# kmaninis/OSVOS-PyTorch

Hardware: NVIDIA H100
Metric: frames/sec at 480x854 fwd-only, batch 1 per GPU (OSVOS.forward -> 5 logit maps) (higher is better)
Workload: dtype bf16x3 (split-bf16 operands, fp32 accumulate)

## Files before the change

osvos_pytorch_b200/csrc/common.cuh:

```cuda
#pragma once
#include <cuda.h>
#include <cuda_bf16.h>
#include <cuda_runtime.h>
#include <stdint.h>
#include <stdio.h>
#include <string.h>

#include "../../include/osvos_b200.h"

namespace osvos {

#define OSVOS_CHECK_ARG(cond)                                                              \
  do {                                                                                     \
    if (!(cond)) {                                                                         \
      set_last_error("%s:%d: invalid argument: %s", __FILE__, __LINE__, #cond);            \
      return OSVOS_ERR_INVALID_ARGUMENT;                                                   \
    }                                                                                      \
  } while (0)

#define OSVOS_CHECK_CUDA(expr)                                                             \
  do {                                                                                     \
    cudaError_t e__ = (expr);                                                              \
    if (e__ != cudaSuccess) {                                                              \
      set_last_error("%s:%d: %s -> %s", __FILE__, __LINE__, #expr, cudaGetErrorString(e__)); \
      return OSVOS_ERR_CUDA;                                                               \
    }                                                                                      \
  } while (0)

void set_last_error(const char* fmt, ...);

int encode_tensor_map(CUtensorMap* map, CUtensorMapDataType dtype, int elem_bytes, int rank, const void* base,
                      const uint64_t* dims, const uint64_t* strides_bytes, const uint32_t* box,
                      CUtensorMapSwizzle swizzle);

int device_sm_count();

bool pdl_enabled();

template <typename... KArgs, typename... Args>
static inline cudaError_t launch_pdl(void (*kern)(KArgs...), dim3 grid, dim3 block, size_t smem, cudaStream_t stream,
                                     Args&&... args) {
  cudaLaunchConfig_t cfg;
  memset(&cfg, 0, sizeof(cfg));
  cfg.gridDim = grid;
  cfg.blockDim = block;
  cfg.dynamicSmemBytes = smem;
  cfg.stream = stream;
  cudaLaunchAttribute attr[1];
  attr[0].id = cudaLaunchAttributeProgrammaticStreamSerialization;
  attr[0].val.programmaticStreamSerializationAllowed = 1;
  cfg.attrs = attr;
  cfg.numAttrs = pdl_enabled() ? 1 : 0;
  return cudaLaunchKernelEx(&cfg, kern, static_cast<KArgs>(args)...);
}

template <typename K>
static inline cudaError_t ensure_dynamic_smem(K kern, int bytes, uint64_t* done_mask) {
  int dev = 0;
  cudaError_t e = cudaGetDevice(&dev);
  if (e != cudaSuccess) return e;
  if (dev < 64 && ((*done_mask >> dev) & 1ull)) return cudaSuccess;
  e = cudaFuncSetAttribute(kern, cudaFuncAttributeMaxDynamicSharedMemorySize, bytes);
  if (e == cudaSuccess && dev < 64) *done_mask |= 1ull << dev;
  return e;
}

__device__ __forceinline__ void split_bf16(float v, __nv_bfloat16& hi, __nv_bfloat16& lo) {
  hi = __float2bfloat16_rn(v);
  lo = __float2bfloat16_rn(v - __bfloat162float(hi));
}
__device__ __forceinline__ uint32_t pack_bf16x2(__nv_bfloat16 a, __nv_bfloat16 b) {
  return static_cast<uint32_t>(__bfloat16_as_ushort(a)) | (static_cast<uint32_t>(__bfloat16_as_ushort(b)) << 16);
}
__device__ __forceinline__ bool last_block_arrives(unsigned int* counter) {
  __shared__ bool is_last;
  __threadfence();
  __syncthreads();
  if (threadIdx.x == 0) is_last = atomicAdd(counter, 1u) == gridDim.x * gridDim.y - 1;
  __syncthreads();
  if (is_last) __threadfence();
  return is_last;
}

template <typename T>
__device__ __forceinline__ T block_ordered_sum(const T* rows, int nrows, size_t stride, T* red ) {
  T t = T(0);
  for (int r = threadIdx.x; r < nrows; r += blockDim.x) t += __ldcg(rows + static_cast<size_t>(r) * stride);
  __syncthreads();
  red[threadIdx.x] = t;
  __syncthreads();
  T s = T(0);
  if (threadIdx.x == 0)
    for (int i = 0; i < static_cast<int>(blockDim.x); ++i) s += red[i];
  return s;
}

__device__ __forceinline__ float bf16_lo_to_float(uint32_t packed) { return __uint_as_float(packed << 16); }
__device__ __forceinline__ float bf16_hi_to_float(uint32_t packed) { return __uint_as_float(packed & 0xFFFF0000u); }

}
```

osvos_pytorch_b200/csrc/conv3x3_halo.cu:

```cuda
#include "conv_common.cuh"

namespace osvos {

constexpr int kHaloRows = kTileH + 2;
constexpr int kPitch = kTileW + 2;

template <int BLOCK_N, int PLANES, bool SPLIT>
struct HaloCfg {
  static constexpr int kABoxBytes = kHaloRows * kPitch * 128;
  static constexpr int kAPlaneBytes = (kABoxBytes + 1023) / 1024 * 1024;
  static constexpr int kAStageBytes = PLANES * kAPlaneBytes;
  static constexpr int kAStages = 2;
  static constexpr int kBPlaneBytes = BLOCK_N * 128;
  static constexpr int kBStageBytes = PLANES * kBPlaneBytes;
  static constexpr int kBudget = 225 * 1024 - kAStages * kAStageBytes;
  static constexpr int kBStagesRaw = kBudget / kBStageBytes;
  static constexpr int kBStages = kBStagesRaw > 9 ? 9 : kBStagesRaw;
  static constexpr bool kSplitAcc = SPLIT;
  static_assert(!SPLIT || (PLANES == 2 && BLOCK_N <= 128), "split accumulators need two planes and 2 * BLOCK_N <= 256");
  static constexpr int kAccCols = kSplitAcc ? 2 * BLOCK_N : BLOCK_N;
  static constexpr int kAcc = kAccCols / 2;
  static constexpr int kSmemBytes = kAStages * kAStageBytes + kBStages * kBStageBytes + 1024 + 512;
  static_assert(kBStages >= 2, "weight ring too shallow");
  static_assert(kSmemBytes <= 227 * 1024, "more than the per-CTA shared memory of sm_90");
  static_assert(kSmemBytes + 4096 < (1 << 18), "descriptor start-address field would overflow");
  static_assert(kBStageBytes % 1024 == 0, "B stage must keep 1024-byte alignment");
};

template <int BLOCK_N, int PLANES, bool SPLIT, bool LEAN, bool PINGPONG, bool DET = false>
__global__ void __launch_bounds__(kConvThreads, 1)
conv3x3_halo_kernel(const __grid_constant__ CUtensorMap map_x_hi, const __grid_constant__ CUtensorMap map_x_lo,
                    const __grid_constant__ CUtensorMap map_w_hi, const __grid_constant__ CUtensorMap map_w_lo,
                    const ConvParams p) {
  using Cfg = HaloCfg<BLOCK_N, PLANES, SPLIT>;
  constexpr int SA = Cfg::kAStages, SB = Cfg::kBStages;
  constexpr int kHalves = PINGPONG ? 2 : 1;
  static_assert(!PINGPONG || kHalves * Cfg::kAcc <= 128, "a ping-pong warpgroup holds the whole tile's accumulator");

  extern __shared__ uint8_t smem_raw[];
  uint8_t* smem = reinterpret_cast<uint8_t*>((reinterpret_cast<uintptr_t>(smem_raw) + 1023) & ~uintptr_t(1023));
  uint8_t* smem_a = smem;
  uint8_t* smem_b = smem + SA * Cfg::kAStageBytes;
  uint64_t* bars = reinterpret_cast<uint64_t*>(smem_b + SB * Cfg::kBStageBytes);
  uint64_t* a_full = bars;
  uint64_t* a_empty = bars + SA;
  uint64_t* b_full = bars + 2 * SA;
  uint64_t* b_empty = bars + 2 * SA + SB;

  const int warp = threadIdx.x >> 5;
  const int lane = threadIdx.x & 31;

  if (warp == 0 && lane == 0) {
    tma_prefetch_desc(&map_x_hi);
    tma_prefetch_desc(&map_w_hi);
    if (PLANES == 2) {
      tma_prefetch_desc(&map_x_lo);
      tma_prefetch_desc(&map_w_lo);
    }
    constexpr uint32_t kReaders = PINGPONG ? 1 : 2;
    for (int i = 0; i < SA; ++i) {
      mbar_init(&a_full[i], 1);
      mbar_init(&a_empty[i], kReaders);
    }
    for (int i = 0; i < SB; ++i) {
      mbar_init(&b_full[i], 1);
      mbar_init(&b_empty[i], kReaders);
    }
    fence_barrier_init();
  }
  __syncthreads();
  pdl_wait();
  pdl_launch_dependents();

  if (warp < 4) {
    if (PINGPONG) setmaxnreg_dec<40>();
    if (warp != 0) return;
    if (elect_one()) {
      int a_stage = 0, b_stage = 0;
      uint32_t a_phase = 0, b_phase = 0;
      const bool skip_a = (p.ablate & 2) != 0, skip_b = (p.ablate & 1) != 0;
      auto issue_a = [&](int x0, int y0, int img, int kc) {
        mbar_wait(&a_empty[a_stage], a_phase ^ 1);
        if (skip_a) {
          mbar_arrive(&a_full[a_stage]);
        } else {
          uint8_t* st = smem_a + a_stage * Cfg::kAStageBytes;
          mbar_arrive_expect_tx(&a_full[a_stage], PLANES * Cfg::kABoxBytes);
          tma_load_4d(&map_x_hi, &a_full[a_stage], st, kc * kBlockK, x0, y0, img);
          if (PLANES == 2) tma_load_4d(&map_x_lo, &a_full[a_stage], st + Cfg::kAPlaneBytes, kc * kBlockK, x0, y0, img);
        }
        if (++a_stage == SA) {
          a_stage = 0;
          a_phase ^= 1;
        }
      };
      int nb = 0, tx = 0, ty = 0, img = 0;
      const int w_first = static_cast<int>(blockIdx.x), w_stride = static_cast<int>(gridDim.x);
      if (w_first < p.total_tiles) {
        decode_tile(p, w_first, nb, tx, ty, img);
        issue_a(tx * kTileW - 1, ty * kTileH - 1, img, 0);
      }
      for (int tile = w_first; tile < p.total_tiles; tile += w_stride) {
        const bool has_next = tile + w_stride < p.total_tiles;
        int nnb = 0, ntx = 0, nty = 0, nimg = 0;
        if (has_next) decode_tile(p, tile + w_stride, nnb, ntx, nty, nimg);
        const int n0 = nb * BLOCK_N;
        for (int kc = 0; kc < p.k_chunks; ++kc) {
          const int c0 = kc * kBlockK;
#pragma unroll
          for (int tap = 0; tap < 9; ++tap) {
            if (tap == 3) {
              if (kc + 1 < p.k_chunks) issue_a(tx * kTileW - 1, ty * kTileH - 1, img, kc + 1);
              else if (has_next) issue_a(ntx * kTileW - 1, nty * kTileH - 1, nimg, 0);
            }
            mbar_wait(&b_empty[b_stage], b_phase ^ 1);
            if (skip_b) {
              mbar_arrive(&b_full[b_stage]);
            } else {
              uint8_t* st = smem_b + b_stage * Cfg::kBStageBytes;
              mbar_arrive_expect_tx(&b_full[b_stage], Cfg::kBStageBytes);
              tma_load_3d(&map_w_hi, &b_full[b_stage], st, c0, n0, tap);
              if (PLANES == 2) tma_load_3d(&map_w_lo, &b_full[b_stage], st + Cfg::kBPlaneBytes, c0, n0, tap);
            }
            if (++b_stage == SB) {
              b_stage = 0;
              b_phase ^= 1;
            }
          }
        }
        nb = nnb, tx = ntx, ty = nty, img = nimg;
      }
    }
    __syncwarp();
  } else {
    if (PINGPONG) setmaxnreg_inc<232>();
    const int wg = (warp - 4) >> 2, wl = warp & 3;
    const bool leader = (threadIdx.x & 127) == 0;
    constexpr uint64_t kDescA = desc_template(16, kPitch * 128, kDescSW128);
    constexpr uint64_t kDescB = desc_template(16, 1024, kDescSW128);
    constexpr uint32_t kLoPlaneA = Cfg::kAPlaneBytes >> 4, kLoPlaneB = Cfg::kBPlaneBytes >> 4;
    constexpr uint32_t kHalfA = (8 * kPitch * 128) >> 4;
    const uint32_t smem_a_u32 = smem_u32(smem_a) + (PINGPONG ? 0 : wg * 8 * kPitch * 128), smem_b_u32 = smem_u32(smem_b);
    const bool skip_mma = (p.ablate & 4) != 0;
    float acc[kHalves][Cfg::kAcc];
    StageRelease pending;
    constexpr int kOwners = PINGPONG ? 2 : 1;
    for (int k = PINGPONG ? wg : 0;; k += kOwners) {
      const int tile = static_cast<int>(blockIdx.x) + k * static_cast<int>(gridDim.x);
      if (tile >= p.total_tiles) break;
      const bool has_next = tile + static_cast<int>(gridDim.x) < p.total_tiles;
      const int a_seq = k * p.k_chunks, b_seq = 9 * a_seq;
      int a_stage = a_seq % SA, b_stage = b_seq % SB;
      uint32_t a_phase = (a_seq / SA) & 1, b_phase = (b_seq / SB) & 1;
      if (PINGPONG && k > 0) named_bar_sync(1 + wg, 256);
#pragma unroll
      for (int h = 0; h < kHalves; ++h)
#pragma unroll
        for (int i = 0; i < Cfg::kAcc; ++i) acc[h][i] = 0.f;
      for (int kc = 0; kc < p.k_chunks; ++kc) {
        mbar_wait(&a_full[a_stage], a_phase);
        const uint64_t da0 = kDescA | static_cast<uint64_t>((smem_a_u32 + a_stage * Cfg::kAStageBytes) >> 4);
#pragma unroll
        for (int tap = 0; tap < 9; ++tap) {
          const uint32_t tap_off = static_cast<uint32_t>(((tap / 3) * kPitch + (tap % 3)) * (128 >> 4));
          mbar_wait(&b_full[b_stage], b_phase);
          if (PINGPONG && tap == 8 && kc == p.k_chunks - 1 && has_next) named_bar_arrive(1 + (wg ^ 1), 256);
          const uint64_t db_hi = kDescB | static_cast<uint64_t>((smem_b_u32 + b_stage * Cfg::kBStageBytes) >> 4);
          wgmma_fence();
#pragma unroll
          for (int h = 0; h < kHalves; ++h) {
            const uint64_t da_hi = da0 + h * kHalfA + tap_off;
            const uint64_t da_lo = da_hi + kLoPlaneA;
            if (skip_mma) continue;
#pragma unroll
            for (int ks = 0; ks < kBlockK / 16; ++ks) {
              if constexpr (Cfg::kSplitAcc) {
                wgmma_bf16<2 * BLOCK_N>(acc[h], da_hi + 2 * ks, db_hi + 2 * ks, 1);
                wgmma_bf16<BLOCK_N>(acc[h], da_lo + 2 * ks, db_hi + 2 * ks, 1);
              } else if constexpr (PLANES == 2) {
                wgmma_bf16<BLOCK_N>(acc[h], da_lo + 2 * ks, db_hi + 2 * ks, 1);
                wgmma_bf16<BLOCK_N>(acc[h], da_hi + 2 * ks, db_hi + kLoPlaneB + 2 * ks, 1);
                wgmma_bf16<BLOCK_N>(acc[h], da_hi + 2 * ks, db_hi + 2 * ks, 1);
              } else {
                wgmma_bf16<BLOCK_N>(acc[h], da_hi + 2 * ks, db_hi + 2 * ks, 1);
              }
            }
          }
          wgmma_commit();
          wgmma_wait<1>();
          pending.release(leader);
          pending.bar_b = &b_empty[b_stage];
          if (tap == 8) pending.bar_a = &a_empty[a_stage];
          if (++b_stage == SB) {
            b_stage = 0;
            b_phase ^= 1;
          }
        }
        if (++a_stage == SA) {
          a_stage = 0;
          a_phase ^= 1;
        }
      }
      wgmma_wait<0>();
#pragma unroll
      for (int h = 0; h < kHalves; ++h) wgmma_fence_operands(acc[h]);
      pending.release(leader);
#pragma unroll
      for (int h = 0; h < kHalves; ++h)
        conv_epilogue<BLOCK_N, Cfg::kSplitAcc, LEAN, DET>(p, acc[h], tile, PINGPONG ? h : wg, wl, lane);
    }
  }
}

template <int BLOCK_N, int PLANES, bool LEAN = false, bool DET = false>
static int launch_halo(const osvos_conv3x3_args* a, cudaStream_t stream) {
  constexpr bool kSplit = PLANES == 2 && BLOCK_N <= 128;
  using Cfg = HaloCfg<BLOCK_N, PLANES, kSplit>;
  ConvParams p;
  fill_conv_params(p, a, BLOCK_N);
  const int sms = device_sm_count();
  CUtensorMap mx_hi, mx_lo, mw_hi, mw_lo;
  {
    const uint64_t dims[4] = {(uint64_t)a->cin, (uint64_t)a->w, (uint64_t)a->h, (uint64_t)a->n};
    const uint64_t strides[3] = {(uint64_t)a->cin * 2, (uint64_t)a->w * a->cin * 2,
                                 (uint64_t)a->h * a->w * a->cin * 2};
    const uint32_t box[4] = {kBlockK, kPitch, kHaloRows, 1};
    int rc = encode_tensor_map(&mx_hi, CU_TENSOR_MAP_DATA_TYPE_BFLOAT16, 2, 4, a->x_hi, dims, strides, box,
                               CU_TENSOR_MAP_SWIZZLE_128B);
    if (rc) return rc;
    rc = encode_tensor_map(&mx_lo, CU_TENSOR_MAP_DATA_TYPE_BFLOAT16, 2, 4, PLANES == 2 ? a->x_lo : a->x_hi, dims,
                           strides, box, CU_TENSOR_MAP_SWIZZLE_128B);
    if (rc) return rc;
  }
  int rc = encode_weight_maps(&mw_hi, &mw_lo, a, BLOCK_N);
  if (rc) return rc;
  const int grid = p.total_tiles < sms ? p.total_tiles : sms;
  constexpr bool kCanPingPong = BLOCK_N == 64 || BLOCK_N == 128;
  const bool pingpong = kCanPingPong && p.total_tiles > 2 * sms;
  auto kern = pingpong ? conv3x3_halo_kernel<BLOCK_N, PLANES, kSplit && BLOCK_N == 64, LEAN, kCanPingPong, DET>
                       : conv3x3_halo_kernel<BLOCK_N, PLANES, kSplit, LEAN, false, DET>;
  static uint64_t attr_done[2] = {0, 0};
  OSVOS_CHECK_CUDA(ensure_dynamic_smem(kern, Cfg::kSmemBytes, &attr_done[pingpong]));
  OSVOS_CHECK_CUDA(launch_pdl(kern, dim3(grid), dim3(kConvThreads), Cfg::kSmemBytes, stream, mx_hi, mx_lo,
                              mw_hi, mw_lo, p));
  return OSVOS_OK;
}

template <bool DET>
static int conv3x3_halo_dispatch(const osvos_conv3x3_args* a, cudaStream_t stream) {
  const bool fast = (a->flags & OSVOS_FLAG_FAST) != 0;
  const bool lean = !fast && !(a->flags & OSVOS_FLAG_RELU_MASK) && a->colsum == nullptr && a->y_f32 == nullptr;
  const int m_tiles = ((a->w + kTileW - 1) / kTileW) * ((a->h + kTileH - 1) / kTileH) * a->n;
  const int sms = device_sm_count();
  const long tiles128 = static_cast<long>(m_tiles) * (a->cout / 128);
  const long waves128 = (tiles128 + sms - 1) / sms;
  const long waves256 = (static_cast<long>(m_tiles) * (a->cout / 256) + sms - 1) / sms;
  if (a->cout == 64 || (waves128 == 1 && tiles128 * 5 <= static_cast<long>(sms) * 3)) {
    if (lean) return launch_halo<64, 2, true>(a, stream);
    return fast ? launch_halo<64, 1, false, DET>(a, stream) : launch_halo<64, 2, false, DET>(a, stream);
  }
  const bool prefer256 = fast ? waves256 * 1100 < waves128 * 700 : waves256 * 2200 < waves128 * 1000;
  if (a->cout % 256 == 0 && prefer256)
    return fast ? launch_halo<256, 1, false, DET>(a, stream) : launch_halo<256, 2, false, DET>(a, stream);
  if (fast) return launch_halo<128, 1, false, DET>(a, stream);
  if (lean) return launch_halo<128, 2, true>(a, stream);
  return launch_halo<128, 2, false, DET>(a, stream);
}

static int check_conv_args(const osvos_conv3x3_args* a) {
  OSVOS_CHECK_ARG(a != nullptr);
  OSVOS_CHECK_ARG(a->n > 0 && a->h > 0 && a->w > 0);
  OSVOS_CHECK_ARG(a->cin >= 64 && a->cin % 64 == 0);
  OSVOS_CHECK_ARG(a->cout == 2 || a->cout == 16 || a->cout == 64 || (a->cout > 0 && a->cout % 128 == 0));
  OSVOS_CHECK_ARG(a->cout != 2 || (a->pq != nullptr && a->y_hi == nullptr && a->y_f32 == nullptr && a->pool_hi == nullptr &&
                                   a->colsum == nullptr && !(a->flags & (OSVOS_FLAG_RELU | OSVOS_FLAG_RELU_MASK))));
  OSVOS_CHECK_ARG(a->cout != 16 || (a->y_hi == nullptr && a->y_lo == nullptr && !(a->flags & OSVOS_FLAG_RELU_MASK)));
  OSVOS_CHECK_ARG(a->x_hi != nullptr && a->w_packed != nullptr);
  OSVOS_CHECK_ARG((a->flags & OSVOS_FLAG_FAST) || a->x_lo != nullptr);
  OSVOS_CHECK_ARG(a->y_hi != nullptr || a->y_f32 != nullptr || a->pq != nullptr || a->pool_hi != nullptr);
  OSVOS_CHECK_ARG(!(a->flags & OSVOS_FLAG_RELU_MASK) || a->mask_hi != nullptr);
  OSVOS_CHECK_ARG(a->pq == nullptr || a->cout == 2 || (a->cout == 16 && a->proj_w != nullptr));
  OSVOS_CHECK_ARG((a->pool_hi == nullptr && a->colsum == nullptr) || a->cout >= 64);
  OSVOS_CHECK_ARG((reinterpret_cast<uintptr_t>(a->x_hi) & 15) == 0);
  OSVOS_CHECK_ARG((reinterpret_cast<uintptr_t>(a->w_packed) & 15) == 0);
  OSVOS_CHECK_ARG((reinterpret_cast<uintptr_t>(a->bias) & 15) == 0);
  OSVOS_CHECK_ARG(!(a->flags & OSVOS_FLAG_DETERMINISTIC) || (reinterpret_cast<uintptr_t>(a->colsum) & 7) == 0);
  if (a->cout >= 64) {
    const uintptr_t bf16_planes = reinterpret_cast<uintptr_t>(a->y_hi) | reinterpret_cast<uintptr_t>(a->y_lo) |
                                  reinterpret_cast<uintptr_t>(a->pool_hi) | reinterpret_cast<uintptr_t>(a->pool_lo) |
                                  reinterpret_cast<uintptr_t>(a->mask_hi);
    OSVOS_CHECK_ARG((bf16_planes & 3) == 0);
    OSVOS_CHECK_ARG((reinterpret_cast<uintptr_t>(a->y_f32) & 7) == 0);
  }
  return OSVOS_OK;
}

}

using namespace osvos;

extern "C" int osvos_side_folded_multi(const osvos_conv3x3_args* args, int count, osvos_stream_t stream_) {
  OSVOS_CHECK_ARG(args != nullptr && count > 0 && count <= 4);
  const osvos_conv3x3_args* order[4];
  for (int k = 0; k < count; ++k) {
    int rc = check_conv_args(&args[k]);
    if (rc) return rc;
    OSVOS_CHECK_ARG(args[k].cout == 2);
    OSVOS_CHECK_ARG((args[k].flags & OSVOS_FLAG_FAST) == (args[0].flags & OSVOS_FLAG_FAST));
    order[k] = &args[k];
  }
  for (int i = 1; i < count; ++i)
    for (int j = i; j > 0 && order[j]->cin > order[j - 1]->cin; --j) {
      const osvos_conv3x3_args* t = order[j];
      order[j] = order[j - 1];
      order[j - 1] = t;
    }
  return side_conv_multi_dispatch(order, count, static_cast<cudaStream_t>(stream_));
}

extern "C" int osvos_conv3x3(const osvos_conv3x3_args* a, osvos_stream_t stream_) {
  int rc = check_conv_args(a);
  if (rc) return rc;
  cudaStream_t stream = static_cast<cudaStream_t>(stream_);
  if (a->cout == 2 || a->cout == 16) return side_conv_dispatch(a, stream);
  if ((a->flags & OSVOS_FLAG_DETERMINISTIC) && a->colsum != nullptr) return conv3x3_halo_dispatch<true>(a, stream);
  return conv3x3_halo_dispatch<false>(a, stream);
}

extern "C" size_t osvos_conv3x3_colsum_rows(int n, int h, int w) {
  if (n <= 0 || h <= 0 || w <= 0) return 0;
  return static_cast<size_t>(n) * ((h + kTileH - 1) / kTileH) * ((w + kTileW - 1) / kTileW) * 8;
}
```

osvos_pytorch_b200/csrc/conv_common.cuh:

```cuda
#pragma once
#include <stdlib.h>

#include "common.cuh"
#include "ptx.cuh"

namespace osvos {

constexpr int kTileW = 8;
constexpr int kTileH = 16;
constexpr int kBlockM = 128;
constexpr int kBlockK = 64;
constexpr int kConvThreads = 384;
constexpr int kABytes = kBlockM * kBlockK * 2;

struct ConvParams {
  const float* bias;
  __nv_bfloat16* y_hi;
  __nv_bfloat16* y_lo;
  float* y_f32;
  const __nv_bfloat16* mask_hi;
  __nv_bfloat16* pool_hi;
  __nv_bfloat16* pool_lo;
  float* colsum;
  int n, h, w, cin, cout;
  int tiles_x, tiles_y, n_blocks, total_tiles, k_chunks;
  int flags;
  int ablate;
};

__device__ __forceinline__ void decode_tile(const ConvParams& p, int tile, int& nb, int& tx, int& ty, int& img) {
  nb = tile % p.n_blocks;
  int m = tile / p.n_blocks;
  tx = m % p.tiles_x;
  m /= p.tiles_x;
  ty = m % p.tiles_y;
  img = m / p.tiles_y;
}

__device__ __forceinline__ uint32_t sw128_offset(int row, int chunk) { return row * 128 + ((chunk ^ (row & 7)) << 4); }

__device__ __forceinline__ void split_pack2(float a, float b, uint32_t& hi, uint32_t& lo) {
  asm("cvt.rn.bf16x2.f32 %0, %1, %2;" : "=r"(hi) : "f"(b), "f"(a));
  const float ra = a - __uint_as_float(hi << 16);
  const float rb = b - __uint_as_float(hi & 0xFFFF0000u);
  asm("cvt.rn.bf16x2.f32 %0, %1, %2;" : "=r"(lo) : "f"(rb), "f"(ra));
}

template <int BLOCK_N, bool SPLIT_ACC, bool LEAN = false, bool DET = false>
__device__ __forceinline__ void conv_epilogue(const ConvParams& p, const float* acc, int tile, int wg, int wl, int lane) {
  if (p.ablate & 16) return;
  int nb, tx, ty, img;
  decode_tile(p, tile, nb, tx, ty, img);
  const int lx = lane >> 2;
  const int x = tx * kTileW + lx;
  const int y0 = ty * kTileH + wg * 8 + wl * 2;
  const bool va = (y0 < p.h) && (x < p.w), vb = (y0 + 1 < p.h) && (x < p.w);
  const bool relu = (p.flags & OSVOS_FLAG_RELU) != 0;
  const bool masked = !LEAN && (p.flags & OSVOS_FLAG_RELU_MASK) != 0;
  const bool store_ok = !(p.ablate & 8);
  const size_t pix[2] = {(static_cast<size_t>(img) * p.h + y0) * p.w + x, (static_cast<size_t>(img) * p.h + y0 + 1) * p.w + x};
  const bool valid[2] = {va, vb};
  const int oh = (p.h + 1) >> 1, ow = (p.w + 1) >> 1;
  const bool pool_writer = va && !(lx & 1) && store_ok;
  const size_t opix = (static_cast<size_t>(img) * oh + (y0 >> 1)) * ow + (x >> 1);
#pragma unroll
  for (int j = 0; j < BLOCK_N / 8; ++j) {
    const int c = 8 * j + 2 * (lane & 3);
    const int ch = nb * BLOCK_N + c;
    const float2 b = p.bias ? __ldg(reinterpret_cast<const float2*>(p.bias + ch)) : make_float2(0.f, 0.f);
    float f[2][2];
#pragma unroll
    for (int h = 0; h < 2; ++h) {
#pragma unroll
      for (int e = 0; e < 2; ++e) {
        float v = e ? b.y : b.x;
        v += acc[4 * j + 2 * h + e];
        if (SPLIT_ACC) v += acc[BLOCK_N / 2 + 4 * j + 2 * h + e];
        f[h][e] = relu ? fmaxf(v, 0.f) : v;
      }
    }
#pragma unroll
    for (int h = 0; h < 2; ++h) {
      if (!LEAN && masked && valid[h]) {
        const uint32_t m = __ldg(reinterpret_cast<const unsigned int*>(p.mask_hi + pix[h] * p.cout + ch));
        if (!(bf16_lo_to_float(m) > 0.f)) f[h][0] = 0.f;
        if (!(bf16_hi_to_float(m) > 0.f)) f[h][1] = 0.f;
      }
      if (valid[h] && store_ok) {
        if (!LEAN && p.y_f32) *reinterpret_cast<float2*>(p.y_f32 + pix[h] * p.cout + ch) = make_float2(f[h][0], f[h][1]);
        if (p.y_hi) {
          uint32_t hi, lo;
          split_pack2(f[h][0], f[h][1], hi, lo);
          *reinterpret_cast<uint32_t*>(p.y_hi + pix[h] * p.cout + ch) = hi;
          if (p.y_lo) *reinterpret_cast<uint32_t*>(p.y_lo + pix[h] * p.cout + ch) = lo;
        }
      }
    }
    if (!LEAN && p.colsum) {
      float s0 = (va ? f[0][0] : 0.f) + (vb ? f[1][0] : 0.f);
      float s1 = (va ? f[0][1] : 0.f) + (vb ? f[1][1] : 0.f);
#pragma unroll
      for (int o = 4; o <= 16; o <<= 1) {
        s0 += __shfl_xor_sync(0xffffffffu, s0, o);
        s1 += __shfl_xor_sync(0xffffffffu, s1, o);
      }
      if (lane < 4) {
        if constexpr (DET) {
          const size_t prow = (static_cast<size_t>(tile / p.n_blocks) * 2 + wg) * 4 + wl;
          *reinterpret_cast<float2*>(p.colsum + prow * p.cout + ch) = make_float2(s0, s1);
        } else {
          atomicAdd(p.colsum + ch, s0);
          atomicAdd(p.colsum + ch + 1, s1);
        }
      }
    }
    if (p.pool_hi) {
      float m0 = fmaxf(va ? f[0][0] : -INFINITY, vb ? f[1][0] : -INFINITY);
      float m1 = fmaxf(va ? f[0][1] : -INFINITY, vb ? f[1][1] : -INFINITY);
      m0 = fmaxf(m0, __shfl_xor_sync(0xffffffffu, m0, 4));
      m1 = fmaxf(m1, __shfl_xor_sync(0xffffffffu, m1, 4));
      if (pool_writer) {
        uint32_t hi, lo;
        split_pack2(m0, m1, hi, lo);
        *reinterpret_cast<uint32_t*>(p.pool_hi + opix * p.cout + ch) = hi;
        if (p.pool_lo) *reinterpret_cast<uint32_t*>(p.pool_lo + opix * p.cout + ch) = lo;
      }
    }
  }
}

constexpr int kStageBoxBytes = 64 * 64 * 2;

struct OutMaps {
  CUtensorMap y_hi, y_lo;
};

__device__ __forceinline__ void conv_epilogue_staged(const ConvParams& p, const OutMaps& maps, const float* acc, int tile,
                                                     int half, int wl, int lane, uint8_t* box, int bar_id, bool leader) {
  if (p.ablate & 16) return;
  int nb, tx, ty, img;
  decode_tile(p, tile, nb, tx, ty, img);
  const int lx = lane >> 2;
  const bool relu = (p.flags & OSVOS_FLAG_RELU) != 0;
  const bool store_ok = !(p.ablate & 8);
  const int planes = p.y_lo ? 2 : 1;
  const uint32_t act_row = smem_u32(box) + (wl * 2 * 8 + lx) * 128;
  const uint32_t col = 4 * (lane & 3);
#pragma unroll 1
  for (int plane = 0; plane < planes; ++plane) {
    if (leader) bulk_wait_group_read<0>();
    named_bar_sync(bar_id, 128);
#pragma unroll
    for (int j = 0; j < 8; ++j) {
      const int ch = nb * 64 + 8 * j + 2 * (lane & 3);
      const float2 b = p.bias ? __ldg(reinterpret_cast<const float2*>(p.bias + ch)) : make_float2(0.f, 0.f);
      float f[2][2];
#pragma unroll
      for (int h = 0; h < 2; ++h) {
#pragma unroll
        for (int e = 0; e < 2; ++e) {
          float v = e ? b.y : b.x;
          v += acc[4 * j + 2 * h + e];
          f[h][e] = relu ? fmaxf(v, 0.f) : v;
        }
      }
#pragma unroll
      for (int h = 0; h < 2; ++h) {
        uint32_t hi, lo;
        split_pack2(f[h][0], f[h][1], hi, lo);
        st_shared_u32(act_row + h * 8 * 128 + ((j ^ lx) << 4) + col, plane ? lo : hi);
      }
    }
    fence_proxy_async_smem();
    named_bar_sync(bar_id, 128);
    if (leader && store_ok) {
      tma_store_4d(plane ? &maps.y_lo : &maps.y_hi, box, nb * 64, tx * kTileW, ty * kTileH + half * 8, img);
      bulk_commit_group();
    }
  }
}


static inline void fill_conv_params(ConvParams& p, const osvos_conv3x3_args* a, int block_n) {
  p.bias = a->bias;
  p.y_hi = static_cast<__nv_bfloat16*>(a->y_hi);
  p.y_lo = static_cast<__nv_bfloat16*>(a->y_lo);
  p.y_f32 = a->y_f32;
  p.mask_hi = static_cast<const __nv_bfloat16*>(a->mask_hi);
  p.pool_hi = static_cast<__nv_bfloat16*>(a->pool_hi);
  p.pool_lo = static_cast<__nv_bfloat16*>(a->pool_lo);
  p.colsum = a->colsum;
  p.n = a->n;
  p.h = a->h;
  p.w = a->w;
  p.cin = a->cin;
  p.cout = a->cout;
  p.tiles_x = (a->w + kTileW - 1) / kTileW;
  p.tiles_y = (a->h + kTileH - 1) / kTileH;
  p.n_blocks = a->cout / block_n;
  p.total_tiles = p.tiles_x * p.tiles_y * a->n * p.n_blocks;
  p.k_chunks = a->cin / kBlockK;
  p.flags = a->flags;
  {
    static int ablate = -1;
    if (ablate < 0) {
      const char* e = getenv("OSVOS_ABLATE");
      ablate = e ? atoi(e) : 0;
    }
    p.ablate = ablate;
  }
}

static inline int encode_weight_maps(CUtensorMap* hi, CUtensorMap* lo, const osvos_conv3x3_args* a, int block_n) {
  const size_t plane = static_cast<size_t>(9) * a->cout * a->cin;
  const uint64_t dims[3] = {(uint64_t)a->cin, (uint64_t)a->cout, 9};
  const uint64_t strides[2] = {(uint64_t)a->cin * 2, (uint64_t)a->cout * a->cin * 2};
  const uint32_t box[3] = {kBlockK, (uint32_t)block_n, 1};
  const __nv_bfloat16* wp = static_cast<const __nv_bfloat16*>(a->w_packed);
  int rc = encode_tensor_map(hi, CU_TENSOR_MAP_DATA_TYPE_BFLOAT16, 2, 3, wp, dims, strides, box,
                             CU_TENSOR_MAP_SWIZZLE_128B);
  if (rc) return rc;
  return encode_tensor_map(lo, CU_TENSOR_MAP_DATA_TYPE_BFLOAT16, 2, 3, wp + plane, dims, strides, box,
                           CU_TENSOR_MAP_SWIZZLE_128B);
}

static inline bool outputs_tma_aligned(const osvos_conv3x3_args* a) {
  return ((reinterpret_cast<uintptr_t>(a->y_hi) | reinterpret_cast<uintptr_t>(a->y_lo)) & 15) == 0;
}

static inline int encode_output_maps(OutMaps* m, const osvos_conv3x3_args* a) {
  memset(m, 0, sizeof(*m));
  const uint64_t c = a->cout;
  const uint64_t dims[4] = {c, (uint64_t)a->w, (uint64_t)a->h, (uint64_t)a->n};
  const uint64_t strides[3] = {c * 2, c * 2 * a->w, c * 2 * a->w * a->h};
  const uint32_t box[4] = {64, kTileW, kTileH / 2, 1};
  int rc = encode_tensor_map(&m->y_hi, CU_TENSOR_MAP_DATA_TYPE_BFLOAT16, 2, 4, a->y_hi, dims, strides, box,
                             CU_TENSOR_MAP_SWIZZLE_128B);
  if (rc == OSVOS_OK && a->y_lo)
    rc = encode_tensor_map(&m->y_lo, CU_TENSOR_MAP_DATA_TYPE_BFLOAT16, 2, 4, a->y_lo, dims, strides, box,
                           CU_TENSOR_MAP_SWIZZLE_128B);
  return rc;
}

int conv_first_tc_launch(const float* x, const float* w_oihw, const float* bias, void* y_hi, void* y_lo, int n, int h,
                         int w, int flags, cudaStream_t stream);
int side_conv_dispatch(const osvos_conv3x3_args* a, cudaStream_t stream);
int side_conv_multi_dispatch(const osvos_conv3x3_args* const* args, int count, cudaStream_t stream);

}
```

osvos_pytorch_b200/csrc/ptx.cuh:

```cuda
#pragma once
#include <cuda.h>
#include <cuda_runtime.h>
#include <stdint.h>

#include "wgmma.cuh"

namespace osvos {

#ifndef OSVOS_SPIN_LIMIT
#define OSVOS_SPIN_LIMIT (1u << 26)
#endif

__device__ __forceinline__ uint32_t smem_u32(const void* p) {
  return static_cast<uint32_t>(__cvta_generic_to_shared(p));
}

__device__ __forceinline__ bool elect_one() {
  uint32_t pred = 0;
  asm volatile(
      "{\n\t.reg .pred P;\n\t"
      "elect.sync _|P, 0xffffffff;\n\t"
      "selp.u32 %0, 1, 0, P;\n\t}\n"
      : "=r"(pred));
  return pred != 0;
}

__device__ __forceinline__ void pdl_wait() { asm volatile("griddepcontrol.wait;" ::: "memory"); }
__device__ __forceinline__ void pdl_launch_dependents() { asm volatile("griddepcontrol.launch_dependents;" ::: "memory"); }

__device__ __forceinline__ void mbar_init(uint64_t* bar, uint32_t count) {
  asm volatile("mbarrier.init.shared::cta.b64 [%0], %1;" ::"r"(smem_u32(bar)), "r"(count) : "memory");
}
__device__ __forceinline__ void fence_barrier_init() {
  asm volatile("fence.mbarrier_init.release.cluster;" ::: "memory");
}
__device__ __forceinline__ void fence_proxy_async_smem() {
  asm volatile("fence.proxy.async.shared::cta;" ::: "memory");
}
__device__ __forceinline__ void mbar_arrive_expect_tx(uint64_t* bar, uint32_t bytes) {
  asm volatile("mbarrier.arrive.expect_tx.shared::cta.b64 _, [%0], %1;" ::"r"(smem_u32(bar)), "r"(bytes)
               : "memory");
}
__device__ __forceinline__ void mbar_arrive(uint64_t* bar) {
  asm volatile("mbarrier.arrive.shared::cta.b64 _, [%0];" ::"r"(smem_u32(bar)) : "memory");
}
__device__ __forceinline__ bool mbar_try_wait(uint64_t* bar, uint32_t parity) {
  uint32_t ok;
  asm volatile(
      "{\n\t.reg .pred P;\n\t"
      "mbarrier.try_wait.parity.shared::cta.b64 P, [%1], %2;\n\t"
      "selp.u32 %0, 1, 0, P;\n\t}\n"
      : "=r"(ok)
      : "r"(smem_u32(bar)), "r"(parity)
      : "memory");
  return ok != 0;
}

__device__ __forceinline__ void mbar_wait(uint64_t* bar, uint32_t parity) {
  uint32_t spins = 0;
  while (!mbar_try_wait(bar, parity)) {
    if (++spins > OSVOS_SPIN_LIMIT) __trap();
  }
}

__device__ __forceinline__ void cp_async_8_zfill(void* dst, const void* src, uint32_t src_bytes) {
  asm volatile("cp.async.ca.shared.global [%0], [%1], 8, %2;" ::"r"(smem_u32(dst)), "l"(src), "r"(src_bytes) : "memory");
}
__device__ __forceinline__ void cp_async_mbar_arrive_noinc(uint64_t* bar) {
  asm volatile("cp.async.mbarrier.arrive.noinc.shared::cta.b64 [%0];" ::"r"(smem_u32(bar)) : "memory");
}

__device__ __forceinline__ void tma_prefetch_desc(const CUtensorMap* m) {
  asm volatile("prefetch.tensormap [%0];" ::"l"(reinterpret_cast<uint64_t>(m)) : "memory");
}
__device__ __forceinline__ void tma_load_4d(const CUtensorMap* m, uint64_t* bar, void* dst, int c0, int c1, int c2,
                                            int c3) {
  asm volatile(
      "cp.async.bulk.tensor.4d.shared::cluster.global.mbarrier::complete_tx::bytes"
      " [%0], [%1, {%3, %4, %5, %6}], [%2];"
      ::"r"(smem_u32(dst)), "l"(reinterpret_cast<uint64_t>(m)), "r"(smem_u32(bar)), "r"(c0), "r"(c1), "r"(c2),
      "r"(c3)
      : "memory");
}
__device__ __forceinline__ void tma_load_2d(const CUtensorMap* m, uint64_t* bar, void* dst, int c0, int c1) {
  asm volatile(
      "cp.async.bulk.tensor.2d.shared::cluster.global.mbarrier::complete_tx::bytes"
      " [%0], [%1, {%3, %4}], [%2];"
      ::"r"(smem_u32(dst)), "l"(reinterpret_cast<uint64_t>(m)), "r"(smem_u32(bar)), "r"(c0), "r"(c1)
      : "memory");
}
__device__ __forceinline__ void tma_load_3d(const CUtensorMap* m, uint64_t* bar, void* dst, int c0, int c1, int c2) {
  asm volatile(
      "cp.async.bulk.tensor.3d.shared::cluster.global.mbarrier::complete_tx::bytes"
      " [%0], [%1, {%3, %4, %5}], [%2];"
      ::"r"(smem_u32(dst)), "l"(reinterpret_cast<uint64_t>(m)), "r"(smem_u32(bar)), "r"(c0), "r"(c1), "r"(c2)
      : "memory");
}
__device__ __forceinline__ void st_shared_u32(uint32_t addr, uint32_t v) {
  asm volatile("st.shared.u32 [%0], %1;" ::"r"(addr), "r"(v) : "memory");
}
__device__ __forceinline__ void tma_store_4d(const CUtensorMap* m, const void* src, int c0, int c1, int c2, int c3) {
  asm volatile(
      "cp.async.bulk.tensor.4d.global.shared::cta.bulk_group [%0, {%2, %3, %4, %5}], [%1];"
      ::"l"(reinterpret_cast<uint64_t>(m)), "r"(smem_u32(src)), "r"(c0), "r"(c1), "r"(c2), "r"(c3)
      : "memory");
}
__device__ __forceinline__ void bulk_commit_group() { asm volatile("cp.async.bulk.commit_group;" ::: "memory"); }
template <int N>
__device__ __forceinline__ void bulk_wait_group_read() { asm volatile("cp.async.bulk.wait_group.read %0;" ::"n"(N) : "memory"); }
template <int N>
__device__ __forceinline__ void bulk_wait_group() { asm volatile("cp.async.bulk.wait_group %0;" ::"n"(N) : "memory"); }

constexpr uint64_t kDescSW128 = 1ull << 62;
__host__ __device__ constexpr uint64_t desc_template(uint32_t lbo_bytes, uint32_t sbo_bytes, uint64_t layout) {
  return (static_cast<uint64_t>((lbo_bytes >> 4) & 0x3FFF) << 16) | (static_cast<uint64_t>((sbo_bytes >> 4) & 0x3FFF) << 32) |
         layout;
}
__device__ __forceinline__ uint64_t make_smem_desc(const void* p, uint32_t lbo_bytes, uint32_t sbo_bytes, uint64_t layout) {
  return desc_template(lbo_bytes, sbo_bytes, layout) | static_cast<uint64_t>((smem_u32(p) >> 4) & 0x3FFF);
}

__device__ __forceinline__ void named_bar_sync(int id, int nthreads) {
  asm volatile("bar.sync %0, %1;" ::"r"(id), "r"(nthreads) : "memory");
}
__device__ __forceinline__ void named_bar_arrive(int id, int nthreads) {
  asm volatile("bar.arrive %0, %1;" ::"r"(id), "r"(nthreads) : "memory");
}

template <int N>
__device__ __forceinline__ void setmaxnreg_dec() { asm volatile("setmaxnreg.dec.sync.aligned.u32 %0;" ::"n"(N)); }
template <int N>
__device__ __forceinline__ void setmaxnreg_inc() { asm volatile("setmaxnreg.inc.sync.aligned.u32 %0;" ::"n"(N)); }

struct StageRelease {
  uint64_t* bar_b = nullptr;
  uint64_t* bar_a = nullptr;
  __device__ __forceinline__ void release(bool leader) {
    if (leader) {
      if (bar_b) mbar_arrive(bar_b);
      if (bar_a) mbar_arrive(bar_a);
    }
    bar_b = bar_a = nullptr;
  }
};

}
```

Baseline: 653.8.

## Pair conv CTAs in 2-clusters and multicast weight slabs via TMA

Launches the 3x3 halo conv as 2-CTA clusters. The two CTAs work on paired spatial tiles that use the same output-channel block, and each CTA loads half of every weight slab and multicasts it to both CTAs' shared memory. Weight-ring empty barriers now count arrivals from both CTAs, signalled through remote mbarrier arrives, and the producer drains the ring before exit so the peer's shared memory stays valid. The goal is to halve weight traffic from L2 per CTA. In exchange the two CTAs of a cluster run in lockstep through the weight ring, an odd tile count leaves ghost tiles that compute without writing, and the grid is sized from the cluster occupancy query.

```diff
diff --git a/osvos_pytorch_b200/csrc/common.cuh b/osvos_pytorch_b200/csrc/common.cuh
--- a/osvos_pytorch_b200/csrc/common.cuh
+++ b/osvos_pytorch_b200/csrc/common.cuh
@@ -54,6 +54,57 @@
   return cudaLaunchKernelEx(&cfg, kern, static_cast<KArgs>(args)...);
 }
 
+template <typename... KArgs, typename... Args>
+static inline cudaError_t launch_pdl_cluster(void (*kern)(KArgs...), int cluster_x, dim3 grid, dim3 block, size_t smem,
+                                             cudaStream_t stream, Args&&... args) {
+  cudaLaunchConfig_t cfg;
+  memset(&cfg, 0, sizeof(cfg));
+  cfg.gridDim = grid;
+  cfg.blockDim = block;
+  cfg.dynamicSmemBytes = smem;
+  cfg.stream = stream;
+  cudaLaunchAttribute attr[2];
+  attr[0].id = cudaLaunchAttributeClusterDimension;
+  attr[0].val.clusterDim.x = cluster_x;
+  attr[0].val.clusterDim.y = 1;
+  attr[0].val.clusterDim.z = 1;
+  attr[1].id = cudaLaunchAttributeProgrammaticStreamSerialization;
+  attr[1].val.programmaticStreamSerializationAllowed = 1;
+  cfg.attrs = attr;
+  cfg.numAttrs = pdl_enabled() ? 2 : 1;
+  return cudaLaunchKernelEx(&cfg, kern, static_cast<KArgs>(args)...);
+}
+
+template <typename K>
+static inline cudaError_t max_active_clusters(K kern, int cluster_x, dim3 block, int smem, int cache[64], int* out) {
+  int dev = 0;
+  cudaError_t e = cudaGetDevice(&dev);
+  if (e != cudaSuccess) return e;
+  if (dev < 64 && cache[dev] > 0) {
+    *out = cache[dev];
+    return cudaSuccess;
+  }
+  cudaLaunchConfig_t cfg;
+  memset(&cfg, 0, sizeof(cfg));
+  cfg.gridDim = dim3(cluster_x);
+  cfg.blockDim = block;
+  cfg.dynamicSmemBytes = smem;
+  cudaLaunchAttribute attr[1];
+  attr[0].id = cudaLaunchAttributeClusterDimension;
+  attr[0].val.clusterDim.x = cluster_x;
+  attr[0].val.clusterDim.y = 1;
+  attr[0].val.clusterDim.z = 1;
+  cfg.attrs = attr;
+  cfg.numAttrs = 1;
+  int n = 0;
+  e = cudaOccupancyMaxActiveClusters(&n, kern, &cfg);
+  if (e != cudaSuccess) return e;
+  if (n <= 0) return cudaErrorInvalidConfiguration;
+  if (dev < 64) cache[dev] = n;
+  *out = n;
+  return cudaSuccess;
+}
+
 template <typename K>
 static inline cudaError_t ensure_dynamic_smem(K kern, int bytes, uint64_t* done_mask) {
   int dev = 0;
diff --git a/osvos_pytorch_b200/csrc/conv3x3_halo.cu b/osvos_pytorch_b200/csrc/conv3x3_halo.cu
--- a/osvos_pytorch_b200/csrc/conv3x3_halo.cu
+++ b/osvos_pytorch_b200/csrc/conv3x3_halo.cu
@@ -12,6 +12,7 @@
   static constexpr int kAStageBytes = PLANES * kAPlaneBytes;
   static constexpr int kAStages = 2;
   static constexpr int kBPlaneBytes = BLOCK_N * 128;
+  static constexpr int kBHalfBytes = kBPlaneBytes / 2;
   static constexpr int kBStageBytes = PLANES * kBPlaneBytes;
   static constexpr int kBudget = 225 * 1024 - kAStages * kAStageBytes;
   static constexpr int kBStagesRaw = kBudget / kBStageBytes;
@@ -25,7 +26,12 @@
   static_assert(kSmemBytes <= 227 * 1024, "more than the per-CTA shared memory of sm_90");
   static_assert(kSmemBytes + 4096 < (1 << 18), "descriptor start-address field would overflow");
   static_assert(kBStageBytes % 1024 == 0, "B stage must keep 1024-byte alignment");
+  static_assert(kBHalfBytes % 1024 == 0, "a half slab must keep the 1024-byte swizzle phase");
 };
+
+__device__ __forceinline__ int pair_tile(const ConvParams& p, int q, uint32_t rank) {
+  return q + static_cast<int>(rank) * p.tile_pairs;
+}
 
 template <int BLOCK_N, int PLANES, bool SPLIT, bool LEAN, bool PINGPONG, bool DET = false>
 __global__ void __launch_bounds__(kConvThreads, 1)
@@ -64,11 +70,12 @@
     }
     for (int i = 0; i < SB; ++i) {
       mbar_init(&b_full[i], 1);
-      mbar_init(&b_empty[i], kReaders);
+      mbar_init(&b_empty[i], 2 * kReaders);
     }
     fence_barrier_init();
   }
-  __syncthreads();
+  cluster_arrive_relaxed();
+  cluster_wait();
   pdl_wait();
   pdl_launch_dependents();
 
@@ -76,6 +83,9 @@
     if (PINGPONG) setmaxnreg_dec<40>();
     if (warp != 0) return;
     if (elect_one()) {
+      const uint32_t rank = blockIdx.x & 1;
+      const int cluster = static_cast<int>(blockIdx.x >> 1), n_clusters = static_cast<int>(gridDim.x >> 1);
+      const int pairs = p.tile_pairs;
       int a_stage = 0, b_stage = 0;
       uint32_t a_phase = 0, b_phase = 0;
       const bool skip_a = (p.ablate & 2) != 0, skip_b = (p.ablate & 1) != 0;
@@ -95,16 +105,15 @@
         }
       };
       int nb = 0, tx = 0, ty = 0, img = 0;
-      const int w_first = static_cast<int>(blockIdx.x), w_stride = static_cast<int>(gridDim.x);
-      if (w_first < p.total_tiles) {
-        decode_tile(p, w_first, nb, tx, ty, img);
+      if (cluster < pairs) {
+        decode_tile(p, pair_tile(p, cluster, rank), nb, tx, ty, img);
         issue_a(tx * kTileW - 1, ty * kTileH - 1, img, 0);
       }
-      for (int tile = w_first; tile < p.total_tiles; tile += w_stride) {
-        const bool has_next = tile + w_stride < p.total_tiles;
+      for (int q = cluster; q < pairs; q += n_clusters) {
+        const bool has_next = q + n_clusters < pairs;
         int nnb = 0, ntx = 0, nty = 0, nimg = 0;
-        if (has_next) decode_tile(p, tile + w_stride, nnb, ntx, nty, nimg);
-        const int n0 = nb * BLOCK_N;
+        if (has_next) decode_tile(p, pair_tile(p, q + n_clusters, rank), nnb, ntx, nty, nimg);
+        const int n0 = nb * BLOCK_N + static_cast<int>(rank) * (BLOCK_N / 2);
         for (int kc = 0; kc < p.k_chunks; ++kc) {
           const int c0 = kc * kBlockK;
 #pragma unroll
@@ -117,10 +126,11 @@
             if (skip_b) {
               mbar_arrive(&b_full[b_stage]);
             } else {
-              uint8_t* st = smem_b + b_stage * Cfg::kBStageBytes;
+              uint8_t* st = smem_b + b_stage * Cfg::kBStageBytes + rank * Cfg::kBHalfBytes;
               mbar_arrive_expect_tx(&b_full[b_stage], Cfg::kBStageBytes);
-              tma_load_3d(&map_w_hi, &b_full[b_stage], st, c0, n0, tap);
-              if (PLANES == 2) tma_load_3d(&map_w_lo, &b_full[b_stage], st + Cfg::kBPlaneBytes, c0, n0, tap);
+              tma_load_3d_multicast(&map_w_hi, &b_full[b_stage], st, c0, n0, tap, 0b11);
+              if (PLANES == 2)
+                tma_load_3d_multicast(&map_w_lo, &b_full[b_stage], st + Cfg::kBPlaneBytes, c0, n0, tap, 0b11);
             }
             if (++b_stage == SB) {
               b_stage = 0;
@@ -129,6 +139,13 @@
           }
         }
         nb = nnb, tx = ntx, ty = nty, img = nimg;
+      }
+      for (int i = 0; i < SB; ++i) {
+        mbar_wait(&b_empty[b_stage], b_phase ^ 1);
+        if (++b_stage == SB) {
+          b_stage = 0;
+          b_phase ^= 1;
+        }
       }
     }
     __syncwarp();
@@ -146,9 +163,10 @@
     StageRelease pending;
     constexpr int kOwners = PINGPONG ? 2 : 1;
     for (int k = PINGPONG ? wg : 0;; k += kOwners) {
-      const int tile = static_cast<int>(blockIdx.x) + k * static_cast<int>(gridDim.x);
-      if (tile >= p.total_tiles) break;
-      const bool has_next = tile + static_cast<int>(gridDim.x) < p.total_tiles;
+      const int q = static_cast<int>(blockIdx.x >> 1) + k * static_cast<int>(gridDim.x >> 1);
+      if (q >= p.tile_pairs) break;
+      const bool has_next = q + static_cast<int>(gridDim.x >> 1) < p.tile_pairs;
+      const bool ghost = pair_tile(p, q, blockIdx.x & 1) >= p.total_tiles;
       const int a_seq = k * p.k_chunks, b_seq = 9 * a_seq;
       int a_stage = a_seq % SA, b_stage = b_seq % SB;
       uint32_t a_phase = (a_seq / SA) & 1, b_phase = (b_seq / SB) & 1;
@@ -188,7 +206,7 @@
           }
           wgmma_commit();
           wgmma_wait<1>();
-          pending.release(leader);
+          pending.release_pair(leader);
           pending.bar_b = &b_empty[b_stage];
           if (tap == 8) pending.bar_a = &a_empty[a_stage];
           if (++b_stage == SB) {
@@ -204,10 +222,12 @@
       wgmma_wait<0>();
 #pragma unroll
       for (int h = 0; h < kHalves; ++h) wgmma_fence_operands(acc[h]);
-      pending.release(leader);
+      pending.release_pair(leader);
+      if (ghost) continue;
 #pragma unroll
       for (int h = 0; h < kHalves; ++h)
-        conv_epilogue<BLOCK_N, Cfg::kSplitAcc, LEAN, DET>(p, acc[h], tile, PINGPONG ? h : wg, wl, lane);
+        conv_epilogue<BLOCK_N, Cfg::kSplitAcc, LEAN, DET>(p, acc[h], pair_tile(p, q, blockIdx.x & 1), PINGPONG ? h : wg,
+                                                          wl, lane);
     }
   }
 }
@@ -232,17 +252,20 @@
                            strides, box, CU_TENSOR_MAP_SWIZZLE_128B);
     if (rc) return rc;
   }
-  int rc = encode_weight_maps(&mw_hi, &mw_lo, a, BLOCK_N);
+  int rc = encode_weight_maps(&mw_hi, &mw_lo, a, BLOCK_N / 2);
   if (rc) return rc;
-  const int grid = p.total_tiles < sms ? p.total_tiles : sms;
   constexpr bool kCanPingPong = BLOCK_N == 64 || BLOCK_N == 128;
   const bool pingpong = kCanPingPong && p.total_tiles > 2 * sms;
   auto kern = pingpong ? conv3x3_halo_kernel<BLOCK_N, PLANES, kSplit && BLOCK_N == 64, LEAN, kCanPingPong, DET>
                        : conv3x3_halo_kernel<BLOCK_N, PLANES, kSplit, LEAN, false, DET>;
   static uint64_t attr_done[2] = {0, 0};
+  static int cluster_cap[2][64];
   OSVOS_CHECK_CUDA(ensure_dynamic_smem(kern, Cfg::kSmemBytes, &attr_done[pingpong]));
-  OSVOS_CHECK_CUDA(launch_pdl(kern, dim3(grid), dim3(kConvThreads), Cfg::kSmemBytes, stream, mx_hi, mx_lo,
-                              mw_hi, mw_lo, p));
+  int clusters = 0;
+  OSVOS_CHECK_CUDA(max_active_clusters(kern, 2, dim3(kConvThreads), Cfg::kSmemBytes, cluster_cap[pingpong], &clusters));
+  if (p.tile_pairs < clusters) clusters = p.tile_pairs;
+  OSVOS_CHECK_CUDA(launch_pdl_cluster(kern, 2, dim3(2 * clusters), dim3(kConvThreads), Cfg::kSmemBytes, stream, mx_hi,
+                                      mx_lo, mw_hi, mw_lo, p));
   return OSVOS_OK;
 }
 
diff --git a/osvos_pytorch_b200/csrc/conv_common.cuh b/osvos_pytorch_b200/csrc/conv_common.cuh
--- a/osvos_pytorch_b200/csrc/conv_common.cuh
+++ b/osvos_pytorch_b200/csrc/conv_common.cuh
@@ -24,6 +24,7 @@
   float* colsum;
   int n, h, w, cin, cout;
   int tiles_x, tiles_y, n_blocks, total_tiles, k_chunks;
+  int tile_pairs;
   int flags;
   int ablate;
 };
@@ -199,6 +200,7 @@
   p.tiles_y = (a->h + kTileH - 1) / kTileH;
   p.n_blocks = a->cout / block_n;
   p.total_tiles = p.tiles_x * p.tiles_y * a->n * p.n_blocks;
+  p.tile_pairs = (p.tiles_x * p.tiles_y * a->n + 1) / 2 * p.n_blocks;
   p.k_chunks = a->cin / kBlockK;
   p.flags = a->flags;
   {
diff --git a/osvos_pytorch_b200/csrc/ptx.cuh b/osvos_pytorch_b200/csrc/ptx.cuh
--- a/osvos_pytorch_b200/csrc/ptx.cuh
+++ b/osvos_pytorch_b200/csrc/ptx.cuh
@@ -44,6 +44,19 @@
 __device__ __forceinline__ void mbar_arrive(uint64_t* bar) {
   asm volatile("mbarrier.arrive.shared::cta.b64 _, [%0];" ::"r"(smem_u32(bar)) : "memory");
 }
+
+template <int RANK>
+__device__ __forceinline__ uint32_t mapa_shared(const void* p) {
+  uint32_t r;
+  asm("mapa.shared::cluster.u32 %0, %1, %2;" : "=r"(r) : "r"(smem_u32(p)), "n"(RANK));
+  return r;
+}
+template <int RANK>
+__device__ __forceinline__ void mbar_arrive_cluster(uint64_t* bar) {
+  asm volatile("mbarrier.arrive.shared::cluster.b64 _, [%0];" ::"r"(mapa_shared<RANK>(bar)) : "memory");
+}
+__device__ __forceinline__ void cluster_arrive_relaxed() { asm volatile("barrier.cluster.arrive.relaxed;" ::: "memory"); }
+__device__ __forceinline__ void cluster_wait() { asm volatile("barrier.cluster.wait.acquire;" ::: "memory"); }
 __device__ __forceinline__ bool mbar_try_wait(uint64_t* bar, uint32_t parity) {
   uint32_t ok;
   asm volatile(
@@ -80,6 +93,15 @@
       " [%0], [%1, {%3, %4, %5, %6}], [%2];"
       ::"r"(smem_u32(dst)), "l"(reinterpret_cast<uint64_t>(m)), "r"(smem_u32(bar)), "r"(c0), "r"(c1), "r"(c2),
       "r"(c3)
+      : "memory");
+}
+__device__ __forceinline__ void tma_load_3d_multicast(const CUtensorMap* m, uint64_t* bar, void* dst, int c0, int c1,
+                                                      int c2, uint16_t cta_mask) {
+  asm volatile(
+      "cp.async.bulk.tensor.3d.shared::cluster.global.mbarrier::complete_tx::bytes.multicast::cluster"
+      " [%0], [%1, {%3, %4, %5}], [%2], %6;"
+      ::"r"(smem_u32(dst)), "l"(reinterpret_cast<uint64_t>(m)), "r"(smem_u32(bar)), "r"(c0), "r"(c1), "r"(c2),
+      "h"(cta_mask)
       : "memory");
 }
 __device__ __forceinline__ void tma_load_2d(const CUtensorMap* m, uint64_t* bar, void* dst, int c0, int c1) {
@@ -142,6 +164,16 @@
     }
     bar_b = bar_a = nullptr;
   }
+  __device__ __forceinline__ void release_pair(bool leader) {
+    if (leader) {
+      if (bar_b) {
+        mbar_arrive_cluster<0>(bar_b);
+        mbar_arrive_cluster<1>(bar_b);
+      }
+      if (bar_a) mbar_arrive(bar_a);
+    }
+    bar_b = bar_a = nullptr;
+  }
 };
 
 }
```

Result: slower. 640.8 (median of 6 runs) (-2.0%).
